# lzzcd001/MeshDiffusion

Hardware: AMD Instinct MI355X
Metric: denoise steps/sec on 64^3x4 DMTet grids (sample-steps/s = n_gpus*batch*steps/wall) (higher is better)
Workload: dtype f16f6 in the Winograd convs behind a GroupNorm (fp16 hi*hi MFMA + MX block-scaled e2m3 cross terms in a K-concatenated scaled MFMA at twice the e4m3 rate; operands and weights equalised per input channel by a power of two: md_wino_equaliser, after the load-time calibration from the measured operand

## Files before the change

### include/meshdiffusion_hip.h

```cpp
#ifndef MESHDIFFUSION_HIP_H
#define MESHDIFFUSION_HIP_H

#include <stdint.h>

#ifdef __cplusplus
extern "C" {
#endif

#define MD_OK 0
#define MD_ERR_BAD_ARG (-1)
#define MD_ERR_UNSUPPORTED (-2)
#define MD_ERR_NO_DEVICE (-3)

#define MD_ABI_VERSION 16

enum {
  MD_CFG_C3_128 = 0,
  MD_CFG_C3_128_K16 = 1,
  MD_CFG_C3_32 = 2,
  MD_CFG_C3_LOW = 3,
  MD_CFG_C3_S2 = 4,
  MD_CFG_G1_128 = 5,
  MD_CFG_G1_128_LOW = 6,
  MD_CFG_G1_64_LOW = 7,
// ... 112 lines not shown
                               int64_t s_row, int64_t s_k, float* eq, void* stream);
int md_wino_operand_ms(const float* x1, const float* x2, int32_t c1, int32_t c2, const float* ac, int32_t silu, int32_t batch, int64_t P,
                       float* ms, void* stream);
int md_wino_prep_f8(const float* x1, const float* x2, int32_t c1, int32_t c2, const float* ac, int32_t silu, int32_t ups,
                    const float* eq, void* t_out, int32_t batch, int32_t D, int32_t H, int32_t W, void* stream);
int64_t md_wino_weight_bytes_f8(int32_t cout, int32_t cin);
int md_wino_pack_weights_f8(const float* w, const float* eq, void* wpk, int32_t cout, int32_t cin, int64_t s_row, int64_t s_k, void* stream);
int md_conv3_wino_f8(const void* t_in, const void* wpk, float* out, const float* bias, int64_t bias_bstride,
                     const float* residual, int64_t res_bstride, double* stats, int32_t batch, int32_t cin, int32_t cout,
                     int32_t D, int32_t H, int32_t W, void* stream);
int md_absmax(const float* x, int64_t n, uint32_t* amax_bits, void* stream);
int md_wino_prep_dual_f6(const float* x, int32_t c, void* t_out, void* u_out, float* sums, float tscale, const uint32_t* amax_bits,
                         int32_t batch, int32_t D, int32_t H, int32_t W, void* stream);
int md_conv3_wino_f6_scaled(const void* t_in, const void* wpk, float* out, const float* bias, int64_t bias_bstride,
                            const float* residual, int64_t res_bstride, double* stats, int32_t batch, int32_t cin, int32_t cout,
                            int32_t D, int32_t H, int32_t W, float out_scale, const uint32_t* amax_bits, void* stream);

int md_wino_prep_f6(const float* x1, const float* x2, int32_t c1, int32_t c2, const float* ac, int32_t silu, int32_t ups,
                    const float* eq, void* t_out, int32_t batch, int32_t D, int32_t H, int32_t W, void* stream);
int md_wino_pack_weights_f6(const float* w, const float* eq, void* wpk, int32_t cout, int32_t cin, int64_t s_row, int64_t s_k, void* stream);
int md_conv3_wino_f6(const void* t_in, const void* wpk, float* out, const float* bias, int64_t bias_bstride,
                     const float* residual, int64_t res_bstride, double* stats, int32_t batch, int32_t cin, int32_t cout,
                     int32_t D, int32_t H, int32_t W, void* stream);

#define MD_WINO_FMT_BF16X3 0
#define MD_WINO_FMT_F16F8 1
#define MD_WINO_FMT_F16F6 2
int md_wino_prep_upsdh(int32_t fmt, const float* x1, const float* x2, int32_t c1, int32_t c2, const float* ac, int32_t silu,
                       const float* eq, void* t_out, int32_t batch, int32_t D, int32_t H, int32_t W, void* stream);
int md_conv3_wino_upsdh(int32_t fmt, const void* t_in, const void* wpk, float* out, const float* bias, int64_t bias_bstride,
                        const float* residual, int64_t res_bstride, double* stats, int32_t batch, int32_t cin, int32_t cout,
                        int32_t D, int32_t H, int32_t W, void* stream);

int md_conv3_stem(const void* x16, const void* wpk, float* out, const float* bias, const float* residual, double* stats,
                  int32_t batch, int32_t cout, int32_t D, int32_t H, int32_t W, void* stream);

int md_conv3_head(const float* x, const float* ac, const void* wpk, float* y, int32_t batch, int32_t cin, int32_t rows_alloc,
                  int32_t D, int32_t H, int32_t W, void* stream);

enum { MD_PACK_WPK = 0, MD_PACK_WINO = 1, MD_PACK_WINO_F6 = 2 };
typedef struct MdPackJob {
  const float* w;
  void* out;
  int64_t s_row, s_k, s_tap, n_items, block0;
  int32_t rows, kdim, taps, nt, kc, prec, flip, kind;
} MdPackJob;
int md_pack_batch(const MdPackJob* jobs_dev, int32_t n_jobs, int64_t total_blocks, int32_t tiled, void* stream);

int md_conv3_s2(const float* x, const void* wpk, float* out, const float* bias, int64_t bias_bstride, double* stats,
                int32_t batch, int32_t cin, int32_t rows, int32_t rows_alloc, int32_t D, int32_t H, int32_t W, void* stream);

int md_wino_prep_v2(const float* x1, const float* x2, int32_t c1, int32_t c2, const float* ac, int32_t silu, int32_t ups,
                    void* t_out, int32_t batch, int32_t D, int32_t H, int32_t W, float drop_p, uint64_t drop_seed, void* stream);

int md_wino_prep_dual(const float* x1, const float* x2, int32_t c1, int32_t c2, const float* ac, int32_t silu, int32_t ups,
                      void* t_out, void* u_out, float* sums, int32_t batch, int32_t D, int32_t H, int32_t W, float drop_p,
                      uint64_t drop_seed, void* stream);

int md_attn_fwd(const void* qk, const void* vT, void* out, const float* bias_v, int32_t batch, int32_t C,
                int32_t N, float scale, void* stream);

int md_ancestral_step(const float* x, const float* eps, const float* z, const float* mask,
                      const float* coef, float* x_out, float* x_mean_out, int32_t batch,
                      int32_t C, int64_t P, void* stream);
int md_ddim_step(const double* x, const float* eps, const float* mask, const double* coef, const float* partial,
                 const float* pmask, int32_t ch, double* x_out, double* x0_out, float* x_f32, int32_t batch,
// ... 105 lines not shown
```

### meshdiffusion_amd/_lib.py

```python
import ctypes as C
import os

_HERE = os.path.dirname(os.path.abspath(__file__))
LIB_PATH = os.environ.get("MD_LIB") or os.path.join(_HERE, "libmeshdiffusion_hip.so")

(CFG_C3_128, CFG_C3_128_K16, CFG_C3_32, CFG_C3_LOW, CFG_C3_S2, CFG_G1_128, CFG_G1_128_LOW, CFG_G1_64_LOW,
 CFG_C3_128_V2, CFG_C3_128_SW, CFG_C3_128_PIPE) = range(11)
(CFG_C3_128_FAST, CFG_C5_128_K16, CFG_C5_32_K16, CFG_C3_128_W4, CFG_C3X_32, CFG_C5X_32_K16, CFG_C3X_128_K16, CFG_C5X_128,
 CFG_G1_128_N128) = range(14, 23)
OUT_F32B, OUT_S16B, OUT_NCDHW = 0, 1, 2
PREC_BF16X3, PREC_FP16X2 = 0, 1
A_PACKED, A_S16B = 0, 1
B_S16B, B_F32B_GN = 0, 1
CORRECTOR_LANGEVIN, CORRECTOR_ALD = 0, 1
SDE_REVERSE_DIFFUSION, SDE_EULER_MARUYAMA = 0, 1
LANGEVIN_SLABS = 64

CFG_NT_KC = {
    CFG_C3_128: (128, 32), CFG_C3_128_K16: (128, 16), CFG_C3_32: (32, 32), CFG_C3_LOW: (128, 32),
    CFG_C3_S2: (128, 32), CFG_G1_128: (128, 32), CFG_G1_128_LOW: (128, 32), CFG_G1_64_LOW: (64, 32),
    CFG_C3_128_V2: (128, 32), CFG_C3_128_SW: (128, 32), CFG_C3_128_PIPE: (128, 32),
    CFG_C3_128_FAST: (128, 32), CFG_C5_128_K16: (128, 16), CFG_C5_32_K16: (32, 16), CFG_C3_128_W4: (128, 32), CFG_C3X_32: (32, 32), CFG_C5X_32_K16: (32, 16), CFG_C3X_128_K16: (128, 16), CFG_C5X_128: (128, 32), CFG_G1_128_N128: (128, 32),
}
ABLATION_CFG_NT_KC = {c: (128, 32) for c in (101, 102, 103, 104, 105, 111, 113, 114, 116, 117, 118, 122)}
# ... 36 lines not shown
    "md_gn_stats": (C.c_int, [_P, _P, _I32, _I32, _I64, _I32, _I32, _P]),
    "md_gn_finalize": (C.c_int, [_P, _P, _P, _P, _I32, _I32, _I32, _I64, _F, _P, _P]),
    "md_gn_apply": (C.c_int, [_P, _P, _P, _P, _I32, _I32, _I64, _I32, _I32, _I32, _I32, _F, _U64, _P]),
    "md_dropout_scale": (C.c_int, [_P, _I32, _I32, _I64, _I32, _I32, _F, _U64, _P]),
    "md_zero": (C.c_int, [_P, _I64, _P]),
    "md_timestep_embedding": (C.c_int, [_P, _P, _I32, _I32, _P]),
    "md_linear": (C.c_int, [_P, _P, _P, _P, _I32, _I32, _I32, _I32, _P]),
    "md_ncdhw_to_s16b_xfold": (C.c_int, [_P, _P, _I32, _I32, _I32, _I32, _I32, _I32, _I32, _P]),
    "md_fold_dx": (C.c_int, [_P, _P, _P, _I32, _I32, _I32, _I32, _I32, _I32, _I32, _P]),
    "md_ncdhw_to_s16b": (C.c_int, [_P, _P, _I32, _I32, _I32, _I64, _P]),
    "md_f32b_to_ncdhw": (C.c_int, [_P, _P, _I32, _I32, _I64, _P]),
    "md_ncdhw_to_f32b": (C.c_int, [_P, _P, _I32, _I32, _I64, _P]),
    "md_s16b_to_ncdhw": (C.c_int, [_P, _P, _I32, _I32, _I64, _P]),
    "md_nin_f32": (C.c_int, [_P, _P, _I32, _I32, _P, _P, _P, _I32, _I32, _I64, _I32, _P]),
    "md_wino_operand_bytes": (_I64, [_I32, _I32, _I32, _I32, _I32]),
    "md_wino_prep": (C.c_int, [_P, _P, _I32, _I32, _P, _I32, _I32, _P, _I32, _I32, _I32, _I32, _F, _U64, _P]),
    "md_wino_weight_bytes": (_I64, [_I32, _I32]),
    "md_wino_pack_weights": (C.c_int, [_P, _P, _I32, _I32, _I64, _I64, _I32, _P]),
    "md_conv3_wino": (C.c_int, [_P, _P, _P, _P, _I64, _P, _I64, _P, _I32, _I32, _I32, _I32, _I32, _I32, _I32, _P]),
    "md_wino_equaliser": (C.c_int, [_P, _P, _P, _I32, _I32, _I64, _I64, _P, _P]),
    "md_wino_equaliser_measured": (C.c_int, [_P, _P, _P, _P, _I32, _I32, _I64, _I64, _P, _P]),
    "md_wino_operand_ms": (C.c_int, [_P, _P, _I32, _I32, _P, _I32, _I32, _I64, _P, _P]),
    "md_wino_prep_f8": (C.c_int, [_P, _P, _I32, _I32, _P, _I32, _I32, _P, _P, _I32, _I32, _I32, _I32, _P]),
    "md_wino_weight_bytes_f8": (_I64, [_I32, _I32]),
    "md_wino_pack_weights_f8": (C.c_int, [_P, _P, _P, _I32, _I32, _I64, _I64, _P]),
    "md_conv3_wino_f8": (C.c_int, [_P, _P, _P, _P, _I64, _P, _I64, _P, _I32, _I32, _I32, _I32, _I32, _I32, _P]),
    "md_absmax": (C.c_int, [_P, _I64, _P, _P]),
    "md_wino_prep_dual_f6": (C.c_int, [_P, _I32, _P, _P, _P, _F, _P, _I32, _I32, _I32, _I32, _P]),
    "md_conv3_wino_f6_scaled": (C.c_int, [_P, _P, _P, _P, _I64, _P, _I64, _P, _I32, _I32, _I32, _I32, _I32, _I32, _F, _P, _P]),
    "md_wino_prep_f6": (C.c_int, [_P, _P, _I32, _I32, _P, _I32, _I32, _P, _P, _I32, _I32, _I32, _I32, _P]),
    "md_wino_pack_weights_f6": (C.c_int, [_P, _P, _P, _I32, _I32, _I64, _I64, _P]),
    "md_conv3_wino_f6": (C.c_int, [_P, _P, _P, _P, _I64, _P, _I64, _P, _I32, _I32, _I32, _I32, _I32, _I32, _P]),
    "md_wino_prep_upsdh": (C.c_int, [_I32, _P, _P, _I32, _I32, _P, _I32, _P, _P, _I32, _I32, _I32, _I32, _P]),
    "md_conv3_wino_upsdh": (C.c_int, [_I32, _P, _P, _P, _P, _I64, _P, _I64, _P, _I32, _I32, _I32, _I32, _I32, _I32, _P]),
    "md_conv3_stem": (C.c_int, [_P, _P, _P, _P, _P, _P, _I32, _I32, _I32, _I32, _I32, _P]),
    "md_conv3_head": (C.c_int, [_P, _P, _P, _P, _I32, _I32, _I32, _I32, _I32, _I32, _P]),
    "md_pack_batch": (C.c_int, [_P, _I32, _I64, _I32, _P]),
    "md_conv3_s2": (C.c_int, [_P, _P, _P, _P, _I64, _P, _I32, _I32, _I32, _I32, _I32, _I32, _I32, _P]),
    "md_wino_prep_v2": (C.c_int, [_P, _P, _I32, _I32, _P, _I32, _I32, _P, _I32, _I32, _I32, _I32, _F, _U64, _P]),
    "md_wino_prep_dual": (C.c_int, [_P, _P, _I32, _I32, _P, _I32, _I32, _P, _P, _P, _I32, _I32, _I32, _I32, _F, _U64, _P]),
    "md_wgrad_wino_workspace_bytes": (_I64, [_I32, _I32, _I32]),
    "md_wgrad_wino": (C.c_int, [_P, _P, _P, _P, _I64, _I32, _I32, _I32, _I32, _I32, _I32, _I32, _I64, _I64, _I64, _P]),
    "md_wgrad_nin_workspace_bytes": (_I64, [_I32, _I32, _I32]),
    "md_wgrad_nin": (C.c_int, [_P, _P, _P, _P, _I64, _I32, _I32, _I32, _I64, _I32, _I64, _I64, _P]),
    "md_attn_fwd": (C.c_int, [_P, _P, _P, _P, _I32, _I32, _I32, _F, _P]),
    "md_softmax_keys": (C.c_int, [_P, _P, _I32, _I32, _I32, _P]),
    "md_ancestral_step": (C.c_int, [_P, _P, _P, _P, _P, _P, _P, _I32, _I32, _I64, _P]),
    "md_ddim_step": (C.c_int, [_P, _P, _P, _P, _P, _P, _I32, _P, _P, _P, _I32, _I32, _I64, _P]),
    "md_langevin_norms": (C.c_int, [_P, _P, _I32, _I32, _I64, _P, _P]),
    "md_langevin_step": (C.c_int, [_P, _P, _P, _P, _P, _P, _F, _I32, _P, _P, _P, _I32, _I32, _I64, _P]),
    "md_sde_step": (C.c_int, [_P, _P, _P, _P, _P, _I32, _P, _P, _I32, _I32, _I64, _P]),
    "md_inpaint_blend": (C.c_int, [_P, _P, _P, _P, _I32, _I32, _I32, _I64, _I64, _P]),
    "md_inpaint_renoise": (C.c_int, [_P, _P, _P, _P, _P, _P, _I32, _I32, _I32, _I64, _P]),
    "md_ddpm_perturb": (C.c_int, [_P, _P, _P, _P, _P, _I32, _I32, _I64, _P]),
    "md_masked_sq_err": (C.c_int, [_P, _P, _P, _P, _P, _F, _I32, _I32, _I64, _P]),
    "md_grad_sqnorm": (C.c_int, [_P, _I64, _P, _P]),
    "md_adam_ema_step": (C.c_int, [_P, _P, _P, _P, _P, _I64, _F, _F, _F, _F, _F, _I32, _F, _P, _F, _P]),
    "md_pb16_bytes": (_I64, [_I32, _I32, _I32, _I32, _I32, _I32, _I32]),
    "md_to_pb16": (C.c_int, [_P, _P, _I32, _I32, _I32, _I32, _I32, _I32, _I32, _I32, _I32, _I32, _I32, _I32, _I32, _P]),
    "md_wgrad_finish": (C.c_int, [_P, _P, _I32, _I32, _I32, _I32, _I32, _I64, _I64, _I64, _P]),
    "md_wgrad_workspace_bytes": (_I64, [_I32, _I32, _I32, _I32]),
    "md_wgrad": (C.c_int, [_P, _P, _P, _P, _I64, _I32, _I32, _I32, _I32, _I32, _I32, _I32, _I32, _I32, _I32, _I32, _I64, _I64,
                           _I64, _P]),
    "md_gn_bwd_stats": (C.c_int, [_P, _P, _P, _P, _I32, _I32, _I64, _I32, _I32, _I32, _I32, _F, _U64, _P]),
    "md_gn_bwd_finalize": (C.c_int, [_P, _P, _P, _P, _P, _P, _I32, _I32, _I32, _I64, _P]),
    "md_gn_bwd_apply": (C.c_int, [_P, _P, _P, _P, _P, _I32, _I32, _I64, _I32, _I32, _I32, _I32, _I32, _F, _U64, _P, _P, _P, _P]),
# ... 76 lines not shown
```

### meshdiffusion_amd/csrc/wino_prep2.hip

```cpp
#include "md_common.h"

namespace {
constexpr int P2_POS = 256;
constexpr int P2_STRIDE = 12;
constexpr int P2_REGION = (P2_POS / 2) * P2_STRIDE + 16;
constexpr int P2_GROUP = 2 * P2_REGION;
#ifdef P2_OLD_IMAGE
__device__ __forceinline__ int p2_slot(int p) { return p * P2_STRIDE; }
#else
__device__ __forceinline__ int p2_slot(int p) { return (p & 1) * P2_REGION + (p >> 1) * P2_STRIDE; }
#endif
}

template <bool DUAL, bool F8 = false>
__global__ __launch_bounds__(256) void md_wino_prep2_kernel(const float* __restrict__ x1, const float* __restrict__ x2,
                                                            int c1, int c2, const float* __restrict__ ac, int silu, int ups,
                                                            uint4* __restrict__ T, uint4* __restrict__ U, float* __restrict__ sums,
                                                            int batch, int D, int H, int W, uint32_t thr16, float drop_scale,
                                                            uint64_t seed, const float* __restrict__ eq) {
  __shared__ __attribute__((aligned(16))) float act[P2_GROUP];
  __shared__ float wsum[32];
  float psum[8];
  const int tid = threadIdx.x;
  const int Wp = W >> 1;
// ... 358 lines not shown
  hipLaunchKernelGGL(md_wino_prep2_f6_kernel<true>, dim3((unsigned)blocks), dim3(256), 0, (hipStream_t)stream, x, (const float*)nullptr, c, 0,
                     (const float*)nullptr, 0, 0, (uint4*)t_out, batch, D, H, W, (const float*)nullptr, (uint4*)u_out, sums, tscale, amax_bits);
  MD_HIP_CHECK_LAUNCH();
  return MD_OK;
}

extern "C" int md_wino_prep_upsdh(int32_t fmt, const float* x1, const float* x2, int32_t c1, int32_t c2, const float* ac, int32_t silu,
                                  const float* eq, void* t_out, int32_t batch, int32_t D, int32_t H, int32_t W, void* stream) {
  if (fmt < MD_WINO_FMT_BF16X3 || fmt > MD_WINO_FMT_F16F6) return MD_ERR_BAD_ARG;
  const int cmask = fmt == MD_WINO_FMT_F16F6 ? 15 : 7;
  if (!x1 || !t_out || batch <= 0 || c1 <= 0 || c2 < 0 || (c1 & cmask) || (c2 & cmask) || (c2 > 0 && !x2)) return MD_ERR_BAD_ARG;
  if ((eq && fmt == MD_WINO_FMT_BF16X3) || (silu && !ac)) return MD_ERR_BAD_ARG;
  if (D <= 0 || H <= 0 || W <= 0 || ((D | H | W) & 1)) return MD_ERR_BAD_ARG;
  D >>= 1; H >>= 1;
  const int64_t P = (int64_t)D * H * W;
  if ((P2_POS % W) || (P % P2_POS)) return MD_ERR_UNSUPPORTED;
  const int64_t blocks = (int64_t)batch * ((c1 + c2) / (cmask + 1)) * (P / P2_POS);
  if (blocks > 0x7fffffff) return MD_ERR_UNSUPPORTED;
  const dim3 grid((unsigned)blocks);
  hipStream_t st = (hipStream_t)stream;
  MD_HIP_CLEAR_ERROR();
  if (fmt == MD_WINO_FMT_F16F6)
    hipLaunchKernelGGL(md_wino_prep2_f6_kernel<false>, grid, dim3(256), 0, st, x1, x2, c1, c2, ac, silu, 2, (uint4*)t_out, batch, D, H, W, eq,
                       (uint4*)nullptr, (float*)nullptr, 1.0f, (const uint32_t*)nullptr);
  else if (fmt == MD_WINO_FMT_F16F8)
    hipLaunchKernelGGL((md_wino_prep2_kernel<false, true>), grid, dim3(256), 0, st, x1, x2, c1, c2, ac, silu, 2, (uint4*)t_out, (uint4*)nullptr,
                       (float*)nullptr, batch, D, H, W, 0u, 1.0f, (uint64_t)0, eq);
  else
    hipLaunchKernelGGL((md_wino_prep2_kernel<false>), grid, dim3(256), 0, st, x1, x2, c1, c2, ac, silu, 2, (uint4*)t_out, (uint4*)nullptr,
                       (float*)nullptr, batch, D, H, W, 0u, 1.0f, (uint64_t)0, (const float*)nullptr);
  MD_HIP_CHECK_LAUNCH();
  return MD_OK;
}
```

### meshdiffusion_amd/hip_ops.py

```python
import ctypes as C
import math
import os

import torch

from . import _lib
from ._lib import (A_PACKED, A_S16B, PREC_BF16X3, PREC_FP16X2, CFG_C3_128, CFG_C3_128_V2, CFG_C3_128_SW, CFG_C3_128_PIPE, CFG_C3_128_FAST, CFG_C5_128_K16, CFG_C5_32_K16, CFG_C3_128_W4, CFG_C3X_32, CFG_C5X_32_K16, CFG_C3X_128_K16, CFG_C5X_128, CFG_G1_128_N128, CFG_C3_128_K16, CFG_C3_32, CFG_C3_LOW, CFG_C3_S2,
                   CFG_G1_128, CFG_G1_128_LOW, CFG_G1_64_LOW, CFG_NT_KC, OUT_F32B, OUT_NCDHW, OUT_S16B,
                   MdGemmConvArgs, check)


CFG_ABL1, CFG_ABL2, CFG_ABL3, CFG_ABL4, CFG_ABL5 = 101, 102, 103, 104, 105
CFG_F1, CFG_F3, CFG_F4, CFG_F6, CFG_F7, CFG_F8 = 111, 113, 114, 116, 117, 118
CFG_FAST_EC = 122
CONV_STAGGER = int(os.environ.get("MD_CONV_STAGGER", "0"))
DEBUG_ACT_FP16 = 2 if os.environ.get("MD_DEBUG_ACT_FP16") == "1" else 0
_MODES = ("bf16x3", "fp16x2", "f16f8", "f16f6")
DEFAULT_PRECISION = os.environ.get("MD_PRECISION", "bf16x3")
FORCE_PRECISION = os.environ.get("MD_FORCE_PRECISION")
WINO_EQ = os.environ.get("MD_WINO_EQ", "1") == "1"
F8_RAW = os.environ.get("MD_F8_RAW", "0") == "1"


def _decode(mode):
# ... 500 lines not shown
_WINO_SCRATCH = {}


def _wino_scratch(n_bf16, device, slot="t"):
    key = (device.type, device.index, torch.cuda.current_stream(device).cuda_stream, slot)
    buf = _WINO_SCRATCH.get(key)
    if buf is None or buf.numel() < n_bf16:
        _WINO_SCRATCH.pop(key, None)
        buf = None
        buf = _WINO_SCRATCH[key] = torch.empty(n_bf16, dtype=torch.bfloat16, device=device)
    return buf[:n_bf16]


def release_scratch():
    _WINO_SCRATCH.clear()


def wino_f8_ok(S, drop=None, keep=False, parts=None, normalised=True):
    if not (WINO_F8 and PRECISION == "bf16x3" and not drop and not keep and 256 % S == 0 and (normalised or F8_RAW)):
        return False
    if WINO_F8 == "f6" and parts is not None and any(c % 16 for _, c in parts):
        return "f8"
    return WINO_F8


PREP_COMPACT_UPS = os.environ.get("MD_PREP_COMPACT_UPS", "1") == "1"


def prep_compact_ok(ups, D, H, W, drop=None, keep=False):
    return bool(PREP_COMPACT_UPS and WINO_PREP_V2 and ups and not drop and not keep and not ((D | H | W) & 1) and 256 % W == 0
                and ((D // 2) * (H // 2) * W) % 256 == 0)


def wino_prep(parts, ac, silu, ups, B, S, drop=None, keep=False, dual=False, sums=None, f8=False, eq=None, tscale=1.0, amax=None, dims=None,
              compact=False):
    lib = _lib.load()
    D, H, W = dims if dims is not None else (S, S, S)
    cin = sum(c for _, c in parts)
    assert 1 <= len(parts) <= 2
    assert not (compact and (dual or keep or drop)), "the compact operand is an inference layout"
    assert eq is None or (f8 and eq.numel() == cin and eq.dtype == torch.float32 and eq.is_cuda), "eq belongs to the f16f8 / f16f6 operand"
    assert ac is not None or not silu, "SiLU is applied together with the folded GroupNorm affine (pass `ac`)"
    nbytes = lib.md_wino_operand_bytes(B, cin, D, H, W)
    if nbytes <= 0:
        raise _lib.MeshDiffusionHipError("md_wino_operand_bytes: unsupported operand shape")
    dev = parts[0][0].device
    if compact:
        assert ups and prep_compact_ok(ups, D, H, W)
        nbytes //= 4
    t = torch.empty(nbytes // 2, dtype=torch.bfloat16, device=dev) if keep else _wino_scratch(nbytes // 2, dev)
    x2, c2 = (parts[1][0], parts[1][1]) if len(parts) == 2 else (None, 0)
    ev = _prof_begin()
    args = (_ptr(parts[0][0]), _ptr(x2), parts[0][1], c2, _ptr(ac), 1 if silu else 0, 1 if ups else 0)
    tail = (B, D, H, W, drop[0] if drop else 0.0, drop[1] if drop else 0, _stream())
    if compact:
        check(lib.md_wino_prep_upsdh(_lib.WINO_FMT["f6" if f8 == "f6" else ("f8" if f8 else False)], *args[:6], _ptr(eq), _ptr(t), B, D, H, W,
                                     _stream()), "md_wino_prep_upsdh")
    elif f8 and dual:
        assert f8 == "f6" and len(parts) == 1 and ac is None and not (ups or keep or drop or eq is not None) and 256 % W == 0
        u = _wino_scratch(nbytes // 2, dev, slot="u")
        check(lib.md_wino_prep_dual_f6(_ptr(parts[0][0]), cin, _ptr(t), _ptr(u), _ptr(sums), float(tscale), _ptr(amax), B, D, H, W, _stream()),
              "md_wino_prep_dual_f6")
    elif f8:
        assert not (dual or keep or drop), "the f16f8 / f16f6 operand is an inference format"
        if f8 == "f6":
            check(lib.md_wino_prep_f6(*args, _ptr(eq), _ptr(t), B, D, H, W, _stream()), "md_wino_prep_f6")
        else:
            check(lib.md_wino_prep_f8(*args, _ptr(eq), _ptr(t), B, D, H, W, _stream()), "md_wino_prep_f8")
    elif dual:
        if 256 % W:
            raise _lib.MeshDiffusionHipError("md_wino_prep_dual needs W | 256")
        u = _wino_scratch(nbytes // 2, dev, slot="u")
        check(lib.md_wino_prep_dual(*args, _ptr(t), _ptr(u), _ptr(sums), *tail), "md_wino_prep_dual")
    else:
        fn = lib.md_wino_prep_v2 if (WINO_PREP_V2 and 256 % W == 0 and (D * H * W) % 256 == 0) else lib.md_wino_prep
        check(fn(*args, _ptr(t), *tail), "md_wino_prep")
    _prof_end(ev, "wino_prep", 0.0, 4.0 * B * cin * (D * H * W // (8 if ups else 1)) + (16.0 if dual else 8.0) * B * cin * (D * H * W // (4 if compact else 1)),
              f"{cin}@{D}x{H}x{W}" + ("/ups" if ups else "") + ("/dual" if dual else "") + (("/f6" if f8 == "f6" else "/f8") if f8 else ""))
    t._md_fmt = ("f6" if f8 == "f6" else "f8") if f8 else False
    t._md_eq = eq.data_ptr() if eq is not None else 0
    t._md_compact = bool(compact)
    return (t, u) if dual else t


WGRAD_WINO = os.environ.get("MD_WGRAD_WINO", "1") == "1"


def wgrad_wino_ok(co, ci, S, B):
# ... 460 lines not shown
```

### meshdiffusion_amd/lib/diffusion/models/layers.py

```python
import math

import numpy as np
import torch
import torch.nn as nn

from .... import hip_ops as ops


def variance_scaling(scale, mode, distribution, in_axis=1, out_axis=0, dtype=torch.float32, device="cpu"):
    def init(shape, dtype=dtype, device=device):
        receptive = np.prod(shape) / shape[in_axis] / shape[out_axis]
        fan_in, fan_out = shape[in_axis] * receptive, shape[out_axis] * receptive
        denom = {"fan_in": fan_in, "fan_out": fan_out, "fan_avg": (fan_in + fan_out) / 2}[mode]
        var = scale / denom
        if distribution == "normal":
            return torch.randn(*shape, dtype=dtype, device=device) * np.sqrt(var)
        if distribution == "uniform":
            return (torch.rand(*shape, dtype=dtype, device=device) * 2.0 - 1.0) * np.sqrt(3 * var)
        raise ValueError("invalid distribution for variance scaling initializer")

    return init


def default_init(scale=1.0):
# ... 70 lines not shown
        ms = measured() if ops.WINO_EQ else None
        if ms is None and not (gn is not None and ops.WINO_EQ):
            return None
        gp = [gn.weight, gn.bias] if gn is not None else []
        if ms is None:
            return layer._cached(f"{name}/wino_eq", [conv.weight] + gp, lambda: ops.wino_equaliser(gn.weight, gn.bias, conv.weight), mark=False)
        return layer._cached(f"{name}/wino_eqm", [conv.weight] + gp + [ms],
                             lambda: ops.wino_equaliser(gn.weight if gn is not None else None, gn.bias if gn is not None else None,
                                                        conv.weight, a2m=ms), mark=False)

    def build(f8=False):
        if f8:
            fmt = "f6" if f8 == "f6" else "f8"
            ms = measured() if ops.WINO_EQ else None
            use_eq = ms is not None or (gn is not None and ops.WINO_EQ)
            deps = [conv.weight] + ([gn.weight, gn.bias] if (use_eq and gn is not None) else []) + ([ms] if ms is not None else [])
            return layer._cached(f"{name}/wino_{fmt}{('m' if ms is not None else 'e') if use_eq else ''}", deps,
                                 lambda: ops.WinoWeightF8(conv.weight, conv.weight.device, fmt, eq=eq()), mark=False)
        return layer._cached(f"{name}/wino", [conv.weight], lambda: ops.WinoWeight(conv.weight, conv.weight.device))
    build.eq, build.measured = eq, measured
    build.owner, build.site = layer, name
    return build


def fused_operand_ok(pw, ups=0):
    cfgs = (ops.CFG_C3_128_FAST,) if ups else (ops.CFG_C3_128_FAST, ops.CFG_C3_LOW)
    return ops.FUSE_GN_APPLY and pw.cfg in cfgs and pw.prec == ops.PREC_BF16X3


def run_conv3(pw, act_s16, B, S_out, *, bias=None, bias_bstride=0, residual=None, res_bstride=None, ups=0,
              out=None, out_mode=ops.OUT_F32B, rows_alloc=None, want_stats=False, b_f32=None, wino=None):
    P = S_out ** 3
    dev = act_s16.device if act_s16 is not None else b_f32["parts"][0][0].device
    rows_alloc = rows_alloc if rows_alloc is not None else ((pw.rows + 7) // 8) * 8
    if out is None:
        out = ops.f32b_empty(B, rows_alloc, P, dev)
    if residual is not None and res_bstride is None:
        res_bstride = rows_alloc * P
    if (b_f32 is not None and wino is not None and out_mode == ops.OUT_F32B and rows_alloc == pw.rows
            and pw.prec == ops.PREC_BF16X3 and ops.wino_ok(pw.rows, pw.kdim, S_out, B)):
        stats = ops.stats_zeros(B, rows_alloc, dev) if want_stats and ops.FUSE_GN_STATS else None
        owner = getattr(wino, "owner", None)
        if ops.CALIBRATE is not None and owner is not None and not b_f32.get("wino_only"):
            ms = ops.wino_operand_ms(b_f32["parts"], b_f32.get("ac"), b_f32.get("silu"), B, b_f32["parts"][0][0].shape[2])
            rec = ops.CALIBRATE.setdefault((id(owner), wino.site), [owner, wino.site, torch.zeros_like(ms), 0])
            rec[2] += ms
            rec[3] += 1
        f8 = (not b_f32.get("wino_only")) and ops.wino_f8_ok(
            S_out, drop=b_f32.get("drop"), keep=bool(b_f32.get("keep")), parts=b_f32["parts"],
            normalised=b_f32.get("ac") is not None
            or (ops.WINO_EQ and hasattr(wino, "measured") and wino.measured() is not None))
        if f8 and owner is not None and wino.site in getattr(owner, "md_bf16x3_sites", ()):
            f8 = False
        compact = (not b_f32.get("wino_only")) and ops.prep_compact_ok(ups, S_out, S_out, S_out, drop=b_f32.get("drop"), keep=bool(b_f32.get("keep")))
        t = ops.wino_prep(b_f32["parts"], b_f32.get("ac"), b_f32.get("silu"), ups, B, S_out, drop=b_f32.get("drop"),
                          keep=bool(b_f32.get("keep")), f8=f8, eq=wino.eq() if f8 and hasattr(wino, "eq") else None, compact=compact)
        if b_f32.get("keep"):
            b_f32["t_out"] = t
        ops.conv3_wino(wino(f8) if f8 else wino(), t, B, S_out, bias=bias, bias_bstride=bias_bstride, residual=residual,
                       res_bstride=res_bstride or 0, stats=stats, out=out)
        if f8 and ops.AUDIT is not None:
            t3 = ops.wino_prep(b_f32["parts"], b_f32.get("ac"), b_f32.get("silu"), ups, B, S_out, compact=compact)
            ref = ops.conv3_wino(wino(), t3, B, S_out, bias=bias, bias_bstride=bias_bstride, residual=residual, res_bstride=res_bstride or 0)
            ops.AUDIT.append(dict(owner=getattr(wino, "owner", None), site=getattr(wino, "site", None), fmt=f8, cin=pw.kdim, cout=pw.rows,
                                  S=S_out, rel_l2=float((torch.linalg.vector_norm(out - ref, dtype=torch.float64)
                                                         / torch.linalg.vector_norm(ref, dtype=torch.float64).clamp_min(1e-300)).item())))
            del t3, ref
        if stats is not None:
            out._md_sums = stats
        elif hasattr(out, "_md_sums"):
            del out._md_sums
        return out
    if b_f32 is not None and b_f32.get("wino_only"):
        b_f32 = None
    ksplit = ops.ksplit_for(pw.cfg, B, pw.rows, pw.kdim, S_out) if out_mode == ops.OUT_F32B else 1
    stats = None
    if (want_stats and ops.FUSE_GN_STATS and ((pw.cfg == ops.CFG_C3_128_FAST and ksplit == 1)
                                              or (ksplit > 1 and ops.SPLITK_STATS and P <= 512 and B * rows_alloc >= 2048))
            and out_mode == ops.OUT_F32B and rows_alloc == pw.rows):
        stats = ops.stats_zeros(B, rows_alloc, dev)
    ops.gemm_conv(cfg=pw.cfg, a=pw.data, b=act_s16, out=out, batch=B, rows=pw.rows,
                  rows_alloc=rows_alloc, kdim=pw.kdim, dims=(S_out, S_out, S_out), bias=bias,
                  bias_bstride=bias_bstride, residual=residual, res_bstride=res_bstride or 0, ups=ups,
                  out_mode=out_mode, ksplit=ksplit, prec=pw.prec, stats=stats, b_f32=b_f32)
    if stats is not None:
        out._md_sums = stats
    elif hasattr(out, "_md_sums"):
        del out._md_sums
    return out


def run_gemm(pw, act_s16, B, P, *, bias=None, bias_bstride=0, residual=None, out=None, out_mode=ops.OUT_F32B,
             alpha=1.0, b_bstride=None, b_f32=None):
    rows_alloc = ((pw.rows + 7) // 8) * 8
    dev = act_s16.device if act_s16 is not None else b_f32["parts"][0][0].device
    if out is None:
        out = (ops.f32b_empty if out_mode == ops.OUT_F32B else ops.s16b_empty)(B, rows_alloc, P, dev)
    return ops.gemm_conv(cfg=pw.cfg, a=pw.data, b=act_s16, out=out, batch=B, rows=pw.rows,
                         rows_alloc=rows_alloc, kdim=pw.kdim, dims=(1, 1, P), bias=bias,
                         bias_bstride=bias_bstride, residual=residual,
                         res_bstride=rows_alloc * P if residual is not None else 0, alpha=alpha,
                         out_mode=out_mode, b_bstride=b_bstride, b_f32=b_f32)


class NIN(HipLayer):

    def __init__(self, in_dim, num_units, init_scale=0.1):
# ... 164 lines not shown
            raise NotImplementedError("conv_shortcut is never enabled by the registered models")
        self.GroupNorm_0 = nn.GroupNorm(num_groups=32, num_channels=in_ch, eps=1e-6)
        self.act = act
        self.Conv_0 = ddpm_conv3x3(in_ch, out_ch)
        if temb_dim is not None:
            self.Dense_0 = nn.Linear(temb_dim, out_ch)
            self.Dense_0.weight.data = default_init()(self.Dense_0.weight.data.shape)
            nn.init.zeros_(self.Dense_0.bias)
        self.GroupNorm_1 = nn.GroupNorm(num_groups=32, num_channels=out_ch, eps=1e-6)
        self.Dropout_0 = nn.Dropout(dropout)
        self.Conv_1 = ddpm_conv3x3(out_ch, out_ch, init_scale=0.0)
        if in_ch != out_ch:
            self.NIN_0 = NIN(in_ch, out_ch)
        self.out_ch, self.in_ch, self.conv_shortcut = out_ch, in_ch, conv_shortcut

    def _bias0(self):
        if hasattr(self, "Dense_0"):
            return self._cached("b0", [self.Conv_0.bias, self.Dense_0.bias],
                                lambda: (self.Conv_0.bias.detach() + self.Dense_0.bias.detach()).contiguous())
        return self.Conv_0.bias

    def forward_blocked(self, parts, B, P, temb=None, bias0=None, bias0_stride=None, tape=None):
        drop = (self.Dropout_0.p, ops.next_dropout_seed()) if self.training and self.Dropout_0.p > 0 else None
        S = _spatial_edge(P)
        cin = sum(c for _, c in parts)
        assert cin == self.in_ch
        cfg = ops.conv_cfg_for(S)
        g0, g1 = self.GroupNorm_0, self.GroupNorm_1
        pw0, pw1 = conv3_packed(self, "w0", self.Conv_0, cfg), conv3_packed(self, "w1", self.Conv_1, cfg)
        f16 = pw0.prec == ops.PREC_FP16X2
        need_nin = self.in_ch != self.out_ch
        if (tape is None and drop is None and fused_operand_ok(pw0) and fused_operand_ok(pw1) and pw0.kdim == cin
                and pw1.kdim == self.out_ch and not ops.NIN_SIDE_STREAM):
            _, ac0 = ops.gn_params(parts, g0.weight, g0.bias, B, P, eps=g0.eps, groups=g0.num_groups, want_ac=True)
            if bias0 is None:
                if temb is not None:
                    bias0, bias0_stride = ops.linear(temb, self.Dense_0.weight, self._bias0(), silu_in=True), self.out_ch
                else:
                    bias0, bias0_stride = self.Conv_0.bias, 0
            h = run_conv3(pw0, None, B, S, bias=bias0, bias_bstride=bias0_stride, want_stats=True,
                          b_f32=dict(parts=parts, ac=ac0, silu=True), wino=conv3_wino_packed(self, "w0", self.Conv_0, gn=g0))
            if need_nin:
                pwn = self.NIN_0.packed(P, hbm_bound=True)
                if pwn.kdim == cin and ops.nin_stream_ok(parts, self.out_ch, P):
                    res = ops.nin_f32(parts, pwn, self.NIN_0.b, B, P)
                elif pwn.cfg in (ops.CFG_G1_128, ops.CFG_G1_128_N128) and pwn.kdim == cin:
                    res = run_gemm(pwn, None, B, P, bias=self.NIN_0.b, b_f32=dict(parts=parts, ac=None, silu=False))
                else:
                    xs = ops.gn_apply(parts, None, B, P, norm=False, silu=False)
                    res = self.NIN_0.forward_s16(xs, B, P)
            else:
                res = parts[0][0]
            _, ac1 = ops.gn_params([(h, self.out_ch)], g1.weight, g1.bias, B, P, eps=g1.eps, groups=g1.num_groups, want_ac=True)
            return run_conv3(pw1, None, B, S, bias=self.Conv_1.bias, residual=res, want_stats=True,
                             b_f32=dict(parts=[(h, self.out_ch)], ac=ac1, silu=True), wino=conv3_wino_packed(self, "w1", self.Conv_1, gn=g1))
        wino_fwd = tape is not None and not f16 and ops.WINO_TRAIN_FWD
        ww0 = wino_fwd and pw0.kdim == cin and ops.wgrad_wino_ok(self.out_ch, cin, S, B)
        ww1 = wino_fwd and pw1.kdim == self.out_ch and ops.wgrad_wino_ok(self.out_ch, self.out_ch, S, B)
        prm, ac0 = ops.gn_params(parts, g0.weight, g0.bias, B, P, eps=g0.eps, groups=g0.num_groups, want_ac=True)
        f0 = dict(parts=parts, ac=ac0, silu=True, wino_only=True, keep=ww0) if wino_fwd else None
        w0 = conv3_wino_packed(self, "w0", self.Conv_0) if f0 is not None else None
        xs = None
        res = None
        if ww0:
            a0 = None
            if need_nin:
                xs = ops.gn_apply(parts, None, B, P, norm=False, silu=False)
        else:
            a0 = ops.gn_apply(parts, prm, B, P, norm=True, silu=True, fp16=f16, want_raw=need_nin)
            if need_nin:
                a0, xs = a0
        if need_nin and ops.NIN_SIDE_STREAM:
            main, side = torch.cuda.current_stream(), ops.side_stream()
            side.wait_stream(main)
            with torch.cuda.stream(side):
                res = self.NIN_0.forward_s16(xs, B, P)
            res.record_stream(main)
            xs.record_stream(side)
        if bias0 is not None:
            h = run_conv3(pw0, a0, B, S, bias=bias0, bias_bstride=bias0_stride, want_stats=True, b_f32=f0, wino=w0)
        elif temb is not None:
            bias0 = ops.linear(temb, self.Dense_0.weight, self._bias0(), silu_in=True)
            h = run_conv3(pw0, a0, B, S, bias=bias0, bias_bstride=self.out_ch, want_stats=True, b_f32=f0, wino=w0)
        else:
            h = run_conv3(pw0, a0, B, S, bias=self.Conv_0.bias, want_stats=True, b_f32=f0, wino=w0)
        prm1, ac1 = ops.gn_params([(h, self.out_ch)], g1.weight, g1.bias, B, P, eps=g1.eps, groups=g1.num_groups, want_ac=True)
        a1 = None if ww1 else ops.gn_apply([(h, self.out_ch)], prm1, B, P, norm=True, silu=True, fp16=f16, drop=drop)
        f1 = dict(parts=[(h, self.out_ch)], ac=ac1, silu=True, drop=drop, wino_only=True, keep=ww1) if wino_fwd else None
# ... 49 lines not shown
```

Baseline: 110.5.

## Add persistent f16f6 Winograd prep kernel that folds GroupNorm finalisation

Adds a persistent-style f16f6 Winograd operand prep kernel. It splits each (batch, channel-pair) unit's position blocks across a resident-sized set of workgroups and double-buffers the next block's load behind the current transform. The kernel can also take raw per-channel GroupNorm sums plus gamma and beta, and compute mean, rstd and the affine coefficients itself. This removes the separate gn_params launch before each ResNet-block conv in inference. In exchange, every workgroup recomputes the group statistics redundantly, and paths that need `ac` (calibration, audit, fallbacks) now resolve it lazily.

New measurement: 110.7 (median of 2 runs). About the same (+0.2%).

```diff
diff --git a/include/meshdiffusion_hip.h b/include/meshdiffusion_hip.h
--- a/include/meshdiffusion_hip.h
+++ b/include/meshdiffusion_hip.h
@@ -168,6 +168,12 @@
                         const float* residual, int64_t res_bstride, double* stats, int32_t batch, int32_t cin, int32_t cout,
                         int32_t D, int32_t H, int32_t W, void* stream);
 
+int md_wino_prep_f6_persist(const float* x1, const float* x2, int32_t c1, int32_t c2, const float* ac, int32_t silu, int32_t ups,
+                            const float* eq, void* t_out, int32_t batch, int32_t D, int32_t H, int32_t W, int32_t wgs_per_unit,
+                            const double* sums1, const double* sums2, const float* gamma, const float* beta, float eps,
+                            int32_t groups, int64_t stat_p, void* stream);
+int md_wino_prep_persist_split(int32_t nblk, int32_t wgs_per_unit, int32_t w, int32_t* b0, int32_t* b1);
+
 int md_conv3_stem(const void* x16, const void* wpk, float* out, const float* bias, const float* residual, double* stats,
                   int32_t batch, int32_t cout, int32_t D, int32_t H, int32_t W, void* stream);
 
diff --git a/meshdiffusion_amd/_lib.py b/meshdiffusion_amd/_lib.py
--- a/meshdiffusion_amd/_lib.py
+++ b/meshdiffusion_amd/_lib.py
@@ -92,6 +92,8 @@
     "md_wino_pack_weights_f6": (C.c_int, [_P, _P, _P, _I32, _I32, _I64, _I64, _P]),
     "md_conv3_wino_f6": (C.c_int, [_P, _P, _P, _P, _I64, _P, _I64, _P, _I32, _I32, _I32, _I32, _I32, _I32, _P]),
     "md_wino_prep_upsdh": (C.c_int, [_I32, _P, _P, _I32, _I32, _P, _I32, _P, _P, _I32, _I32, _I32, _I32, _P]),
+    "md_wino_prep_f6_persist": (C.c_int, [_P, _P, _I32, _I32, _P, _I32, _I32, _P, _P, _I32, _I32, _I32, _I32, _I32, _P, _P, _P, _P, _F, _I32, _I64, _P]),
+    "md_wino_prep_persist_split": (C.c_int, [_I32, _I32, _I32, _P, _P]),
     "md_conv3_wino_upsdh": (C.c_int, [_I32, _P, _P, _P, _P, _I64, _P, _I64, _P, _I32, _I32, _I32, _I32, _I32, _I32, _P]),
     "md_conv3_stem": (C.c_int, [_P, _P, _P, _P, _P, _P, _I32, _I32, _I32, _I32, _I32, _P]),
     "md_conv3_head": (C.c_int, [_P, _P, _P, _P, _I32, _I32, _I32, _I32, _I32, _I32, _P]),
diff --git a/meshdiffusion_amd/csrc/wino_prep2.hip b/meshdiffusion_amd/csrc/wino_prep2.hip
--- a/meshdiffusion_amd/csrc/wino_prep2.hip
+++ b/meshdiffusion_amd/csrc/wino_prep2.hip
@@ -414,3 +414,241 @@
   MD_HIP_CHECK_LAUNCH();
   return MD_OK;
 }
+
+
+__host__ __device__ inline void md_prep_split(int nblk, int wpu, int w, int& b0, int& b1) {
+  const int q = nblk / wpu, r = nblk - q * wpu;
+  b0 = w * q + (w < r ? w : r);
+  b1 = b0 + q + (w < r ? 1 : 0);
+}
+
+namespace {
+struct P2PersistArgs {
+  const float *x1, *x2, *ac, *eq;
+  uint4* T;
+  const double *s1, *s2;
+  const float *gamma, *beta;
+  int64_t stat_p;
+  float eps;
+  int groups, c1, c2, silu, ups, D, H, W, wpu;
+};
+}
+
+template <int ACT>
+__global__ __launch_bounds__(256, 5) void md_wino_prep2_f6_persist_kernel(const P2PersistArgs a) {
+  __shared__ __attribute__((aligned(16))) float act[2 * P2_GROUP];
+  __shared__ __attribute__((aligned(16))) float coef[3][16];
+  const int tid = threadIdx.x;
+  const int H = a.H, W = a.W, c1 = a.c1, c2 = a.c2, ups = a.ups;
+  const int P = a.D * H * W, Ph = P >> 1;
+  const int CG = (c1 + c2) >> 3, CGP = CG >> 1;
+  const int nblk = P / P2_POS;
+  const int w = blockIdx.x % a.wpu, unit = blockIdx.x / a.wpu;
+  const int cgp = unit % CGP, b = unit / CGP;
+  int b0, b1;
+  md_prep_split(nblk, a.wpu, w, b0, b1);
+  const int Hi = ups == 1 ? H >> 1 : H, Wi = ups ? W >> 1 : W;
+  const int64_t Pin = ups == 1 ? (int64_t)(P >> 3) : ups == 2 ? (int64_t)(P >> 1) : (int64_t)P;
+  const float* src = (cgp * 16 < c1) ? a.x1 + ((int64_t)b * (c1 >> 3) + 2 * cgp) * Pin * 8
+                                     : a.x2 + ((int64_t)b * (c2 >> 3) + (2 * cgp - (c1 >> 3))) * Pin * 8;
+  const int x = tid & (W - 1), rl = tid / W, rpb = P2_POS / W;
+  auto load = [&](int blk, f32x4 (&v)[4]) {
+    int spos;
+    if (ups == 0) {
+      spos = blk * P2_POS + tid;
+    } else {
+      const int r = blk * rpb + rl;
+      spos = (ups == 2 ? r : ((r / H) >> 1) * Hi + ((r % H) >> 1)) * Wi + (x >> 1);
+    }
+    const f32x4* sp = (const f32x4*)(src + (int64_t)spos * 8);
+    const f32x4* sq = (const f32x4*)(src + (Pin + spos) * 8);
+    v[0] = sp[0]; v[1] = sp[1]; v[2] = sq[0]; v[3] = sq[1];
+  };
+#ifdef P2P_INTERLEAVE
+  const int step = a.wpu;
+  b1 = w + (b1 - b0) * step;
+  b0 = w;
+#else
+  const int step = 1;
+#endif
+  f32x4 v[4];
+  load(b0, v);
+  const bool has_eq = a.eq != nullptr;
+  if (a.s1 != nullptr) {
+    const int ctot = c1 + c2, cpg = ctot / a.groups, ch0 = cgp * 16;
+    const int g_hi = (ch0 + 15) / cpg;
+    const int lane = tid & 63;
+    for (int g = ch0 / cpg + (tid >> 6); g <= g_hi; g += 4) {
+      double s = 0.0, q = 0.0;
+      for (int c = lane; c < cpg; c += 64) {
+        const int ch = g * cpg + c;
+        const double* sp = ch < c1 ? a.s1 + ((int64_t)b * c1 + ch) * 2 : a.s2 + ((int64_t)b * c2 + (ch - c1)) * 2;
+        s += sp[0];
+        q += sp[1];
+      }
+#pragma unroll
+      for (int o = 32; o > 0; o >>= 1) { s += __shfl_xor(s, o, 64); q += __shfl_xor(q, o, 64); }
+      const double n = (double)cpg * (double)a.stat_p;
+      const double mean = s / n;
+      double var = q / n - mean * mean;
+      if (var < 0.0) var = 0.0;
+      const float rstd = (float)(1.0 / sqrt(var + (double)a.eps));
+      for (int c = lane; c < cpg; c += 64) {
+        const int ch = g * cpg + c;
+        if (ch >= ch0 && ch < ch0 + 16) {
+          const float a_ = rstd * a.gamma[ch];
+          coef[0][ch - ch0] = a_;
+          coef[1][ch - ch0] = (float)((double)a.beta[ch] - mean * (double)a_);
+        }
+      }
+    }
+  } else if (a.ac != nullptr && tid < 16) {
+    const float* ap = a.ac + ((int64_t)b * (c1 + c2) + cgp * 16) * 2;
+    coef[0][tid] = ap[2 * tid];
+    coef[1][tid] = ap[2 * tid + 1];
+  }
+  if (has_eq && tid >= 64 && tid < 80) coef[2][tid - 64] = a.eq[cgp * 16 + tid - 64];
+  __syncthreads();
+  const int pi = tid & 127, fh = __builtin_amdgcn_readfirstlane(tid >> 7);
+  const int lp = 2 * pi, px = lp & (W - 1);
+  bool la[2], lb[2];
+  int sa[2], sb[2];
+#pragma unroll
+  for (int g = 0; g < 2; ++g) {
+    const int ka = fh == 0 ? g : 2 - g, kb = fh == 0 ? 2 : 1 + 2 * g;
+    const int xa = px - 1 + ka, xb = px - 1 + kb;
+    la[g] = xa >= 0 && xa < W;
+    lb[g] = xb >= 0 && xb < W;
+    sa[g] = la[g] ? p2_slot(lp - 1 + ka) : 0;
+    sb[g] = lb[g] ? p2_slot(lp - 1 + kb) : 0;
+  }
+  float* const dst = act + p2_slot(tid);
+  auto stage = [&]() {
+#pragma unroll
+    for (int g2 = 0; g2 < 2; ++g2) {
+      float yv[8];
+#pragma unroll
+      for (int e = 0; e < 8; ++e) yv[e] = e < 4 ? v[2 * g2][e] : v[2 * g2 + 1][e - 4];
+      if constexpr (ACT != 0) {
+#pragma unroll
+        for (int e = 0; e < 8; ++e) {
+          float t = yv[e] * coef[0][g2 * 8 + e] + coef[1][g2 * 8 + e];
+          if constexpr (ACT == 2) t = t * __builtin_amdgcn_rcpf(1.0f + __builtin_amdgcn_exp2f(t * -1.4426950408889634f));
+          yv[e] = t;
+        }
+      }
+      if (has_eq) {
+#pragma unroll
+        for (int e = 0; e < 8; ++e) yv[e] *= coef[2][g2 * 8 + e];
+      }
+      *(f32x4*)(dst + g2 * P2_GROUP) = f32x4{yv[0], yv[1], yv[2], yv[3]};
+      *(f32x4*)(dst + g2 * P2_GROUP + 4) = f32x4{yv[4], yv[5], yv[6], yv[7]};
+    }
+  };
+  uint4* out = a.T + ((int64_t)b * CG + 2 * cgp) * 8 * Ph + (int64_t)(4 * fh) * Ph + ((int64_t)b0 * (P2_POS / 2) + pi);
+  stage();
+  for (int blk = b0;; blk += step) {
+    const bool more = blk + step < b1;
+    if (more) load(blk + step, v);
+    __syncthreads();
+#pragma unroll
+    for (int g = 0; g < 2; ++g) {
+      float t[16];
+#pragma unroll
+      for (int g2 = 0; g2 < 2; ++g2) {
+        f32x4 p0 = {0.f, 0.f, 0.f, 0.f}, p1 = p0, q0 = p0, q1 = p0;
+        if (la[g]) {
+          const float* sv = act + g2 * P2_GROUP + sa[g];
+          p0 = *(const f32x4*)sv; p1 = *(const f32x4*)(sv + 4);
+        }
+        if (lb[g]) {
+          const float* sv = act + g2 * P2_GROUP + sb[g];
+          q0 = *(const f32x4*)sv; q1 = *(const f32x4*)(sv + 4);
+        }
+#pragma unroll
+        for (int e = 0; e < 8; ++e) {
+          const float da = e < 4 ? p0[e] : p1[e - 4], db = e < 4 ? q0[e] : q1[e - 4];
+          t[g2 * 8 + e] = (fh == 0 && g == 1) ? da + db : da - db;
+        }
+      }
+      uint4 h0, h1, r0, r1;
+      md_split_f16f6(t, false, 0, h0, h1, r0, r1);
+      uint4* o = out + (int64_t)(2 * g) * Ph;
+      o[0] = h0;
+      o[(int64_t)8 * Ph] = h1;
+      o[Ph] = r0;
+      o[(int64_t)9 * Ph] = r1;
+    }
+    out += step * (P2_POS / 2);
+    __syncthreads();
+    if (!more) break;
+    stage();
+  }
+}
+
+static int md_prep_persist_resident() {
+  static int cached[64] = {0};
+  int dev = 0;
+  if (hipGetDevice(&dev) != hipSuccess || dev < 0 || dev >= 64) return 0;
+  if (cached[dev] == 0) {
+    int cus = 0, per_cu = 0;
+    if (hipDeviceGetAttribute(&cus, hipDeviceAttributeMultiprocessorCount, dev) != hipSuccess) return 0;
+    if (hipOccupancyMaxActiveBlocksPerMultiprocessor(&per_cu, md_wino_prep2_f6_persist_kernel<2>, 256, 0) != hipSuccess) return 0;
+    if (cus <= 0 || per_cu <= 0) return 0;
+    cached[dev] = cus * per_cu;
+  }
+  return cached[dev];
+}
+
+extern "C" int md_wino_prep_persist_split(int32_t nblk, int32_t wgs_per_unit, int32_t w, int32_t* b0, int32_t* b1) {
+  if (nblk <= 0 || wgs_per_unit <= 0 || !b0 || !b1) return MD_ERR_BAD_ARG;
+  const int wpu = wgs_per_unit < nblk ? wgs_per_unit : nblk;
+  if (w < 0 || w >= wpu) return MD_ERR_BAD_ARG;
+  int lo, hi;
+  md_prep_split(nblk, wpu, w, lo, hi);
+  *b0 = lo;
+  *b1 = hi;
+  return wpu;
+}
+
+extern "C" int md_wino_prep_f6_persist(const float* x1, const float* x2, int32_t c1, int32_t c2, const float* ac, int32_t silu, int32_t ups,
+                                       const float* eq, void* t_out, int32_t batch, int32_t D, int32_t H, int32_t W, int32_t wgs_per_unit,
+                                       const double* sums1, const double* sums2, const float* gamma, const float* beta, float eps,
+                                       int32_t groups, int64_t stat_p, void* stream) {
+  if (!x1 || !t_out || batch <= 0 || c1 <= 0 || c2 < 0 || (c1 & 15) || (c2 & 15) || (c2 > 0 && !x2)) return MD_ERR_BAD_ARG;
+  if (ups < 0 || ups > 2 || wgs_per_unit < 0) return MD_ERR_BAD_ARG;
+  if (sums1) {
+    if (ac || (c2 > 0 && !sums2) || !gamma || !beta || groups <= 0 || ((c1 + c2) % groups) || stat_p <= 0) return MD_ERR_BAD_ARG;
+  } else if (silu && !ac) {
+    return MD_ERR_BAD_ARG;
+  }
+  if (D <= 0 || H <= 0 || W <= 0 || (W & 1) || (ups && ((D | H | W) & 1))) return MD_ERR_BAD_ARG;
+  if (ups == 2) { D >>= 1; H >>= 1; }
+  const int64_t P = (int64_t)D * H * W;
+  if ((P2_POS % W) || (P % P2_POS) || P > 0x7fffffff) return MD_ERR_UNSUPPORTED;
+  const int nblk = (int)(P / P2_POS);
+  const int64_t units = (int64_t)batch * ((c1 + c2) / 16);
+  int64_t wpu = wgs_per_unit;
+  if (wpu == 0) {
+    const int resident = md_prep_persist_resident();
+    if (resident <= 0) return MD_ERR_UNSUPPORTED;
+    wpu = resident / units;
+    if (wpu < 1) wpu = 1;
+  }
+  if (wpu > nblk) wpu = nblk;
+  if (units * wpu > 0x7fffffff) return MD_ERR_UNSUPPORTED;
+  P2PersistArgs a;
+  a.x1 = x1; a.x2 = x2; a.ac = ac; a.eq = eq; a.T = (uint4*)t_out;
+  a.s1 = sums1; a.s2 = sums2; a.gamma = gamma; a.beta = beta; a.stat_p = stat_p; a.eps = eps; a.groups = groups;
+  a.c1 = c1; a.c2 = c2; a.silu = silu; a.ups = ups; a.D = D; a.H = H; a.W = W; a.wpu = (int)wpu;
+  MD_HIP_CLEAR_ERROR();
+  const dim3 grid((unsigned)(units * wpu));
+  if (!ac && !sums1)
+    hipLaunchKernelGGL(md_wino_prep2_f6_persist_kernel<0>, grid, dim3(256), 0, (hipStream_t)stream, a);
+  else if (!silu)
+    hipLaunchKernelGGL(md_wino_prep2_f6_persist_kernel<1>, grid, dim3(256), 0, (hipStream_t)stream, a);
+  else
+    hipLaunchKernelGGL(md_wino_prep2_f6_persist_kernel<2>, grid, dim3(256), 0, (hipStream_t)stream, a);
+  MD_HIP_CHECK_LAUNCH();
+  return MD_OK;
+}
diff --git a/meshdiffusion_amd/hip_ops.py b/meshdiffusion_amd/hip_ops.py
--- a/meshdiffusion_amd/hip_ops.py
+++ b/meshdiffusion_amd/hip_ops.py
@@ -556,15 +556,36 @@
                 and ((D // 2) * (H // 2) * W) % 256 == 0)
 
 
+PREP_PERSIST = os.environ.get("MD_PREP_PERSIST", "1") == "1"
+
+
+def prep_persist_ok(f8, D, H, W, compact=False, drop=None, keep=False, dual=False):
+    rows = (D // 2) * (H // 2) if compact else D * H
+    return bool(f8 == "f6" and not (drop or keep or dual) and 256 % W == 0 and (rows * W) % 256 == 0 and rows * W < 2 ** 31)
+
+
+def gn_part_sums(parts, B, P):
+    lib = _lib.load()
+    out = []
+    for t, c in parts:
+        cs = getattr(t, "_md_sums", None) if FUSE_GN_STATS else None
+        if cs is None:
+            cs = stats_zeros(B, c, t.device)
+            check(lib.md_gn_stats(_ptr(t), _ptr(cs), B, c, P, c, 0, _stream()), "md_gn_stats")
+        out.append(cs)
+    return out
+
+
 def wino_prep(parts, ac, silu, ups, B, S, drop=None, keep=False, dual=False, sums=None, f8=False, eq=None, tscale=1.0, amax=None, dims=None,
-              compact=False):
+              compact=False, gn=None, persist=None, wgs_per_unit=0):
     lib = _lib.load()
     D, H, W = dims if dims is not None else (S, S, S)
     cin = sum(c for _, c in parts)
     assert 1 <= len(parts) <= 2
     assert not (compact and (dual or keep or drop)), "the compact operand is an inference layout"
     assert eq is None or (f8 and eq.numel() == cin and eq.dtype == torch.float32 and eq.is_cuda), "eq belongs to the f16f8 / f16f6 operand"
-    assert ac is not None or not silu, "SiLU is applied together with the folded GroupNorm affine (pass `ac`)"
+    assert ac is not None or gn is not None or not silu, "SiLU is applied together with the folded GroupNorm affine (pass `ac` or `gn`)"
+    assert gn is None or (ac is None and len(gn["sums"]) == len(parts)), "`gn` replaces `ac`: one sum buffer per part"
     nbytes = lib.md_wino_operand_bytes(B, cin, D, H, W)
     if nbytes <= 0:
         raise _lib.MeshDiffusionHipError("md_wino_operand_bytes: unsupported operand shape")
@@ -577,7 +598,17 @@
     ev = _prof_begin()
     args = (_ptr(parts[0][0]), _ptr(x2), parts[0][1], c2, _ptr(ac), 1 if silu else 0, 1 if ups else 0)
     tail = (B, D, H, W, drop[0] if drop else 0.0, drop[1] if drop else 0, _stream())
-    if compact:
+    if persist is None:
+        persist = PREP_PERSIST
+    if gn is not None or (persist and f8 == "f6" and not dual):
+        if not prep_persist_ok(f8, D, H, W, compact=compact, drop=drop, keep=keep, dual=dual):
+            raise _lib.MeshDiffusionHipError("md_wino_prep_f6_persist: not an inference f16f6 operand on a grid of the two-phase pass")
+        gs = list(gn["sums"]) + [None] if gn is not None else [None, None]
+        check(lib.md_wino_prep_f6_persist(*args[:6], 2 if compact else (1 if ups else 0), _ptr(eq), _ptr(t), B, D, H, W, int(wgs_per_unit),
+                                          _ptr(gs[0]), _ptr(gs[1]), _ptr(gn["gamma"]) if gn else None, _ptr(gn["beta"]) if gn else None,
+                                          float(gn["eps"]) if gn else 0.0, int(gn["groups"]) if gn else 0, int(gn["P"]) if gn else 0,
+                                          _stream()), "md_wino_prep_f6_persist")
+    elif compact:
         check(lib.md_wino_prep_upsdh(_lib.WINO_FMT["f6" if f8 == "f6" else ("f8" if f8 else False)], *args[:6], _ptr(eq), _ptr(t), B, D, H, W,
                                      _stream()), "md_wino_prep_upsdh")
     elif f8 and dual:
diff --git a/meshdiffusion_amd/lib/diffusion/models/layers.py b/meshdiffusion_amd/lib/diffusion/models/layers.py
--- a/meshdiffusion_amd/lib/diffusion/models/layers.py
+++ b/meshdiffusion_amd/lib/diffusion/models/layers.py
@@ -126,6 +126,11 @@
               out=None, out_mode=ops.OUT_F32B, rows_alloc=None, want_stats=False, b_f32=None, wino=None):
     P = S_out ** 3
     dev = act_s16.device if act_s16 is not None else b_f32["parts"][0][0].device
+
+    def resolve_ac():
+        g = b_f32.get("gn") if b_f32 is not None else None
+        if g is not None and b_f32.get("ac") is None:
+            b_f32["ac"] = ops.gn_params(b_f32["parts"], g["gamma"], g["beta"], B, g["P"], eps=g["eps"], groups=g["groups"], want_ac=True)[1]
     rows_alloc = rows_alloc if rows_alloc is not None else ((pw.rows + 7) // 8) * 8
     if out is None:
         out = ops.f32b_empty(B, rows_alloc, P, dev)
@@ -135,6 +140,8 @@
             and pw.prec == ops.PREC_BF16X3 and ops.wino_ok(pw.rows, pw.kdim, S_out, B)):
         stats = ops.stats_zeros(B, rows_alloc, dev) if want_stats and ops.FUSE_GN_STATS else None
         owner = getattr(wino, "owner", None)
+        if ops.CALIBRATE is not None or ops.AUDIT is not None:
+            resolve_ac()
         if ops.CALIBRATE is not None and owner is not None and not b_f32.get("wino_only"):
             ms = ops.wino_operand_ms(b_f32["parts"], b_f32.get("ac"), b_f32.get("silu"), B, b_f32["parts"][0][0].shape[2])
             rec = ops.CALIBRATE.setdefault((id(owner), wino.site), [owner, wino.site, torch.zeros_like(ms), 0])
@@ -142,13 +149,19 @@
             rec[3] += 1
         f8 = (not b_f32.get("wino_only")) and ops.wino_f8_ok(
             S_out, drop=b_f32.get("drop"), keep=bool(b_f32.get("keep")), parts=b_f32["parts"],
-            normalised=b_f32.get("ac") is not None
+            normalised=b_f32.get("ac") is not None or b_f32.get("gn") is not None
             or (ops.WINO_EQ and hasattr(wino, "measured") and wino.measured() is not None))
         if f8 and owner is not None and wino.site in getattr(owner, "md_bf16x3_sites", ()):
             f8 = False
         compact = (not b_f32.get("wino_only")) and ops.prep_compact_ok(ups, S_out, S_out, S_out, drop=b_f32.get("drop"), keep=bool(b_f32.get("keep")))
+        gn = None
+        if b_f32.get("gn") is not None and b_f32.get("ac") is None:
+            if ops.PREP_PERSIST and ops.prep_persist_ok(f8, S_out, S_out, S_out, compact=compact, drop=b_f32.get("drop"), keep=bool(b_f32.get("keep"))):
+                gn = dict(b_f32["gn"], sums=ops.gn_part_sums(b_f32["parts"], B, b_f32["gn"]["P"]))
+            else:
+                resolve_ac()
         t = ops.wino_prep(b_f32["parts"], b_f32.get("ac"), b_f32.get("silu"), ups, B, S_out, drop=b_f32.get("drop"),
-                          keep=bool(b_f32.get("keep")), f8=f8, eq=wino.eq() if f8 and hasattr(wino, "eq") else None, compact=compact)
+                          keep=bool(b_f32.get("keep")), f8=f8, eq=wino.eq() if f8 and hasattr(wino, "eq") else None, compact=compact, gn=gn)
         if b_f32.get("keep"):
             b_f32["t_out"] = t
         ops.conv3_wino(wino(f8) if f8 else wino(), t, B, S_out, bias=bias, bias_bstride=bias_bstride, residual=residual,
@@ -167,6 +180,7 @@
         return out
     if b_f32 is not None and b_f32.get("wino_only"):
         b_f32 = None
+    resolve_ac()
     ksplit = ops.ksplit_for(pw.cfg, B, pw.rows, pw.kdim, S_out) if out_mode == ops.OUT_F32B else 1
     stats = None
     if (want_stats and ops.FUSE_GN_STATS and ((pw.cfg == ops.CFG_C3_128_FAST and ksplit == 1)
@@ -397,14 +411,18 @@
         need_nin = self.in_ch != self.out_ch
         if (tape is None and drop is None and fused_operand_ok(pw0) and fused_operand_ok(pw1) and pw0.kdim == cin
                 and pw1.kdim == self.out_ch and not ops.NIN_SIDE_STREAM):
-            _, ac0 = ops.gn_params(parts, g0.weight, g0.bias, B, P, eps=g0.eps, groups=g0.num_groups, want_ac=True)
+            def gn_operand(ps, g):
+                if ops.PREP_PERSIST:
+                    return dict(parts=ps, gn=dict(gamma=g.weight, beta=g.bias, eps=g.eps, groups=g.num_groups, P=P), silu=True)
+                return dict(parts=ps, ac=ops.gn_params(ps, g.weight, g.bias, B, P, eps=g.eps, groups=g.num_groups, want_ac=True)[1], silu=True)
+            f0 = gn_operand(parts, g0)
             if bias0 is None:
                 if temb is not None:
                     bias0, bias0_stride = ops.linear(temb, self.Dense_0.weight, self._bias0(), silu_in=True), self.out_ch
                 else:
                     bias0, bias0_stride = self.Conv_0.bias, 0
             h = run_conv3(pw0, None, B, S, bias=bias0, bias_bstride=bias0_stride, want_stats=True,
-                          b_f32=dict(parts=parts, ac=ac0, silu=True), wino=conv3_wino_packed(self, "w0", self.Conv_0, gn=g0))
+                          b_f32=f0, wino=conv3_wino_packed(self, "w0", self.Conv_0, gn=g0))
             if need_nin:
                 pwn = self.NIN_0.packed(P, hbm_bound=True)
                 if pwn.kdim == cin and ops.nin_stream_ok(parts, self.out_ch, P):
@@ -416,9 +434,8 @@
                     res = self.NIN_0.forward_s16(xs, B, P)
             else:
                 res = parts[0][0]
-            _, ac1 = ops.gn_params([(h, self.out_ch)], g1.weight, g1.bias, B, P, eps=g1.eps, groups=g1.num_groups, want_ac=True)
             return run_conv3(pw1, None, B, S, bias=self.Conv_1.bias, residual=res, want_stats=True,
-                             b_f32=dict(parts=[(h, self.out_ch)], ac=ac1, silu=True), wino=conv3_wino_packed(self, "w1", self.Conv_1, gn=g1))
+                             b_f32=gn_operand([(h, self.out_ch)], g1), wino=conv3_wino_packed(self, "w1", self.Conv_1, gn=g1))
         wino_fwd = tape is not None and not f16 and ops.WINO_TRAIN_FWD
         ww0 = wino_fwd and pw0.kdim == cin and ops.wgrad_wino_ok(self.out_ch, cin, S, B)
         ww1 = wino_fwd and pw1.kdim == self.out_ch and ops.wgrad_wino_ok(self.out_ch, self.out_ch, S, B)
```
